# pdrebello/flash-attention-minitorch

Hardware: AMD Instinct MI355X
Metric: attn fw+bw TFLOP/s at (B=8,H=8,N=4096,d=64); % MFMA roofline (higher is better)
Workload: dtype bf16

## Files before the change

### flash_attention_minitorch_amd/csrc/fa_api.hip

```cpp
#include <hip/hip_runtime.h>
#include <math.h>
#include <algorithm>
#include <chrono>
#include <mutex>
#include <string>
#include <vector>
#include <stdio.h>
#include <stdlib.h>
#include <string.h>
#include <unistd.h>
#include <atomic>

#include "../../include/flash_attn_mi355x.h"
#include "fa_kernels.h"

namespace {

thread_local char g_err[512] = "";

int set_err(int code, const char* what, hipError_t e = hipSuccess) {
  if (e != hipSuccess)
    snprintf(g_err, sizeof(g_err), "%s: %s", what, hipGetErrorString(e));
  else
    snprintf(g_err, sizeof(g_err), "%s", what);
// ... 193 lines not shown
    m.check = false;
    s.add(Kern(base + 2), batch, 256, nqb, 0).twin_blocks = m.twin_blocks;
  }
}

template <typename T, int D>
Selection select_fwd(const Call& c) {
  constexpr bool BF = sizeof(T) == 2;
  const int batch = c.batch, N = c.N, causal = c.causal;
  const Tun& tun = c.tun;
  const bool plain = !c.lay.kmask && !c.lay.drop_thr;
  Selection s;
  if (!BF && D == 64) {
    const long wgs = (long)batch * ((N + 127) / 128), cus = device_cus();
    if (plain && !c.lay.out_bf16 && N >= 128 && (tun.v[1] == 4 ||
         (tun.v[1] == 0 && wgs <= (causal ? FWD_SPLITK_MAX_WGS_PER_CU_CAUSAL : FWD_SPLITK_MAX_WGS_PER_CU) * cus))) {
      const int nqb = (N + 31) / 32;
      s.add(FWD_SPLITK, batch * nqb, 256, nqb);
      return s;
    }
  }
  if (BF && (D == 64 || D == 128)) {
    const int nqb = (N + 255) / 256;
    const bool cslot = causal && N % 256 == 0 && (tun.v[1] == 3 || (tun.v[1] == 0 && batch * nqb >= 256));
    if (c.variant == FA_VARIANT_FA2 && tun.v[1] != 2 && (!causal || tun.v[1] == 3 || cslot) && plain && N >= 64) {
      if (cslot) {
        const bool ranked = causal_ranked(tun, batch * nqb, D == 64 ? 2 : 1);
        s.add(FWD_SLOT_CAUSAL, ranked ? batch * nqb : batch * ((nqb + 1) / 2), 512, nqb, ranked ? 2 : 1).rank_chunk =
            rank_chunk(D == 64 ? 2 : 1, nqb);
        s.folds = true;
        return s;
      }
      if (!causal && N % (8192 / D) == 0) {
        s.add(FWD_SLOT_WHOLE, batch * nqb, 512, nqb, causal);
        s.folds = s.produces_guard = true;
        return s;
      }
      if (D == 64) {
        s.add(FWD_SLOT_MASKED, batch * nqb, 512, nqb, causal);
        if (causal) select_phased(s, c, BF, FWD_DROP, 0, 0, 0, false);
        return s;
      }
    }
  }
  select_phased(s, c, BF, FWD_DROP, -1, D == 64 ? 1 : 0, tun.v[7] == 2 || (tun.v[7] == 0 && BF && D == 32), false);
  return s;
}

template <typename T, int D>
void select_dkdv_phased(Selection& s, const Call& c, bool mode3 = false, int care_main = 0, int rank_causal = 1) {
  constexpr bool BF = sizeof(T) == 2;
  constexpr int NW = BF ? 8 : 4;
  const int batch = c.batch, N = c.N, causal = c.causal;
  const int nkb = (N + NW * 32 - 1) / (NW * 32), nkb4 = (N + 127) / 128;
  const bool rank = causal && rank_causal;
  if (c.lay.drop_thr) {
    if (BF) s.add(DKDV_CARE_DROP, batch * nkb4, 256, nkb4).rank_chunk = rank ? rank_chunk(2, nkb4) : 0;
    else s.add(DKDV_DROP_F32, batch * nkb, NW * 64, nkb).rank_chunk = rank ? rank_chunk(2, nkb) : 0;
    return;
  }
  if (BF && (c.lay.kmask || N < 64)) {
    s.add(DKDV_CARE, batch * nkb4, 256, nkb4).rank_chunk = rank ? rank_chunk(2, nkb4) : 0;
    return;
  }
  if (mode3 && causal && care_main) {
    s.add(DKDV_CARE_MAIN, batch * ((nkb + 1) / 2), NW * 64, nkb);
    return;
// ... 149 lines not shown
#define FA_FWD_SLOT(...) FA_GO((fa::fwd_slot_kernel<__VA_ARGS__>), FA_QKV, c.out, c.l, N, s.nb, batch, lay, s.arg, c.tau)
#define FA_DQ(FEAT, NWQ, ...)                                                                                                    \
  FA_GO((fa::bwd_dq_kernel<T, D, 32, FEAT, NWQ, ##__VA_ARGS__>), FA_QKV, (const T*)c.dout, c.nlc(), c.delta(), c.dq, N, s.nb, batch, lay, \
        causal, c.tau, s.arg, pa)
#define FA_DQ_SLOT(...)                                                                                                            \
  FA_GO((fa::bwd_dq_slot_kernel<T, D, ##__VA_ARGS__>), FA_QKV, (const T*)c.dout, c.nlc(), c.delta(), c.dq, N, s.nb, batch, lay, s.arg, \
        c.tau, pa)
#define FA_DKDV_SLOT(...)                                                                                                         \
  FA_GO((fa::bwd_dkdv_slot_kernel<T, 64, ##__VA_ARGS__>), FA_QKV, (const T*)c.dout, c.nl2(), c.delta(), c.dk, c.dv, N, s.nb, batch, lay, \
        c.tau)
#define FA_DKDV(...)                                                                                                               \
  FA_GO((fa::bwd_dkdv_kernel<T, D, 32, __VA_ARGS__>), FA_QKV, (const T*)c.dout, c.nlc(), c.delta(), c.dk, c.dv, N, s.nb, batch, lay, \
        causal, c.tau, s.arg)
#define FA_ONEPASS(C, R)                                                                                                         \
  FA_GO((fa::bwd_onepass_f32_kernel<D, C, R>), FA_QKV, (const T*)c.dout, c.nlc(), c.delta(), c.dq, c.dk, c.dv, N, s.nb, batch, lay, \
        c.tau, s.arg)
  for (int i = 0; i < sel.n; ++i) {
    const Step& s = sel.steps[i];
    fa::Layout lay = c.lay;
    lay.rank_chunk = s.rank_chunk;
    lay.tiles = s.tiles;
    lay.twin_blocks = s.twin_blocks;
    lay.guard_want = s.guard_want;
    const fa::DqPrep pa = s.prep ? fa::DqPrep{c.out, c.l, c.m, c.nlc(), c.delta(), c.nl2(), c.variant, 1.0f / c.tau} : fa::DqPrep{};
    switch (s.kern) {
      case FWD_SPLITK:
        if constexpr (!BF && D == 64)
          FA_GO((fa::fwd_splitk_f32_kernel<D>), FA_QKV, c.out, c.l, c.m, N, s.nb, batch, lay, causal, c.variant, c.tau);
        break;
      case FWD_SLOT_CAUSAL:
        if constexpr (BF && D >= 64) FA_FWD_SLOT(T, D, false, 64, (D == 64 ? 4 : 2), true);
        break;
      case FWD_SLOT_WHOLE:
        if constexpr (BF && D == 64) FA_FWD_SLOT(T, 64, false, 64, 4);
        else if constexpr (BF && D == 128) FA_FWD_SLOT(T, D, false);
        break;
      case FWD_SLOT_MASKED:
        if constexpr (BF && D == 64) FA_FWD_SLOT(T, D, true);
        break;
      case FWD_DROP: FA_FWD(2, BF); break;
      case FWD_MASK: FA_FWD(1, BF); break;
      case FWD_CARE: FA_FWD(0, BF); break;
      case FWD_MAIN: FA_FWD(0, false); break;
      case BWD_PREP:
        FA_GO((fa::bwd_prep_kernel<T, D>), c.out, (const T*)c.dout, c.l, c.m, c.nlc(), c.delta(), c.nl2(), rows, N, lay, c.variant,
              1.0f / c.tau);
        break;
      case DQ_DROP: FA_DQ(2, 4, BF); break;
      case DQ_MASK: FA_DQ(1, 4, BF); break;
      case DQ_CARE: FA_DQ(0, 4, BF); break;
      case DQ_MAIN: FA_DQ(0, 4, false); break;
      case DQ_WAVE8:
        if constexpr (BF && D == 128) FA_DQ(0, 8);
        break;
      case DQ_SLOT_CAUSAL:
        if constexpr (BF && D == 64) FA_DQ_SLOT(false, true);
        break;
      case DQ_SLOT_TILED:
        if constexpr (BF && D == 64) FA_DQ_SLOT(false, false, true);
        break;
      case DQ_SLOT_WHOLE:
        if constexpr (BF && D == 64) FA_DQ_SLOT(false);
        break;
      case DQ_SLOT_MASKED:
        if constexpr (BF && D == 64) FA_DQ_SLOT();
        break;
      case DKDV_SLOT_TILED:
// ... 851 lines not shown
```

### flash_attention_minitorch_amd/csrc/fa_common.h

```cpp
#pragma once
#include <type_traits>

#include "fa_atoms.h"

namespace fa {

constexpr float LOG2E = 1.4426950408889634f;
constexpr int AUX_FA1 = 1;
constexpr int AUX_FA2 = 2;

template <int V> using ic = std::integral_constant<int, V>;

FA_DEV int lane_fresh() {
  int l;
  asm volatile("v_mbcnt_lo_u32_b32 %0, -1, 0\n\tv_mbcnt_hi_u32_b32 %0, -1, %0" : "=v"(l));
  return l;
}

template <typename T> FA_DEV typename Atom<T>::frag load_frag_buf(rsrc_t rs, int byte_off);
template <> FA_DEV bf16x8 load_frag_buf<bf16_t>(rsrc_t rs, int byte_off) {
  return __builtin_bit_cast(bf16x8, __builtin_amdgcn_raw_buffer_load_b128(rs, byte_off, 0, 0));
}
template <> FA_DEV f32x8 load_frag_buf<float>(rsrc_t rs, int byte_off) {
  f32x4 a = __builtin_bit_cast(f32x4, __builtin_amdgcn_raw_buffer_load_b128(rs, byte_off, 0, 0));
  f32x4 b = __builtin_bit_cast(f32x4, __builtin_amdgcn_raw_buffer_load_b128(rs, byte_off + 16, 0, 0));
  return __builtin_shufflevector(a, b, 0, 1, 2, 3, 4, 5, 6, 7);
}

constexpr int GUARD_SLOTS = 256;
FA_DEV bool guard_beyond(const Layout& L) {
  const int lane = threadIdx.x & 63;
  const f32x4 a = *reinterpret_cast<const f32x4*>(L.guard + 4 * lane);
  const f32x4 b = *reinterpret_cast<const f32x4*>(L.guard + GUARD_SLOTS + 4 * lane);
  float qm = fmaxf(fmaxf(a[0], a[1]), fmaxf(a[2], a[3])), km = fmaxf(fmaxf(b[0], b[1]), fmaxf(b[2], b[3]));
#pragma unroll
  for (int off = 32; off > 0; off >>= 1) {
    qm = fmaxf(qm, __shfl_xor(qm, off));
    km = fmaxf(km, __shfl_xor(km, off));
  }
  const bool beyond = !(L.guard_coef * __builtin_sqrtf(qm * km) <= 1.0f);
  return __builtin_amdgcn_readfirstlane((int)beyond) != 0;
}
FA_DEV bool guard_skip(const Layout& L) {
  if (L.guard == nullptr || L.guard_want >= 2) return false;
  return guard_beyond(L) != (L.guard_want != 0);
}
FA_DEV bool scale_exact(const Layout& L) {
  if (L.scale_sel != 2 || L.guard == nullptr) return L.scale_sel != 0;
  return guard_beyond(L);
}

FA_DEV bool guard_produce(const Layout& L, float qs, float ks, lds_char* scratch) {
  qs = xhalf_sum(qs);
  ks = xhalf_sum(ks);
#pragma unroll
  for (int off = 16; off > 0; off >>= 1) {
    qs = fmaxf(qs, __shfl_xor(qs, off));
    ks = fmaxf(ks, __shfl_xor(ks, off));
  }
  const int w = threadIdx.x >> 6;
  if ((threadIdx.x & 63) == 0) {
    unsigned* g = reinterpret_cast<unsigned*>(const_cast<float*>(L.guard)) + (blockIdx.x & (GUARD_SLOTS - 1));
    atomicMax(g, __float_as_uint(qs));
    atomicMax(g + GUARD_SLOTS, __float_as_uint(ks));
    *FA_LDS(float, scratch + 4 * w) = qs;
    *FA_LDS(float, scratch + 32 + 4 * w) = ks;
  }
  __syncthreads();
  float qm = 0.f, km = 0.f;
#pragma unroll
  for (int i = 0; i < 8; ++i) {
    qm = fmaxf(qm, *FA_LDS(float, scratch + 4 * i));
    km = fmaxf(km, *FA_LDS(float, scratch + 32 + 4 * i));
  }
  __syncthreads();
  return !(L.guard_coef * __builtin_sqrtf(qm * km) <= 1.0f);
}
template <typename F> FA_DEV float frag_sumsq(const F& f) {
  float s = 0.f;
#pragma unroll
  for (int j = 0; j < 8; ++j) s = __builtin_fmaf((float)f[j], (float)f[j], s);
  return s;
}

FA_DEV void store_out4(float* o, size_t elem_off, const f32x4& val, int out_bf16) {
  if (out_bf16) {
    *reinterpret_cast<bf16x4*>(reinterpret_cast<bf16_t*>(o) + elem_off) = __builtin_convertvector(val, bf16x4);
  } else {
    *reinterpret_cast<f32x4*>(o + elem_off) = val;
  }
}

FA_DEV f32x16 zero16() {
  f32x16 z;
#pragma unroll
  for (int i = 0; i < 16; ++i) z[i] = 0.f;
  return z;
}

}
```

### flash_attention_minitorch_amd/csrc/fa_fwd.h

```cpp
#pragma once
#include "fa_common.h"

namespace fa {

constexpr float MAX_DEFER_SUM = 64.0f;

template <typename T, int D, int BN, int WPE, int FEAT = 0, bool CARE = false>
__global__ void __launch_bounds__(256) __attribute__((amdgpu_waves_per_eu(WPE)))
fwd_kernel(const T* __restrict__ q, const T* __restrict__ k, const T* __restrict__ v, float* __restrict__ o,
           float* __restrict__ aux_l, float* __restrict__ aux_m, int N, int nqb, int BH, Layout lay, int causal,
           int aux_mode, float tau, int only_qb = -1) {
  if (guard_skip(lay)) return;
  using A = Atom<T>;
  typedef typename A::frag frag;
  constexpr bool HM = FEAT >= 1, HD = FEAT >= 2;
  constexpr int KC = D / 16, KT = BN / 32, DT = D / 32;
  constexpr int TB = A::template tile_bytes<D>(BN);
  __shared__ __attribute__((aligned(16))) char smem_raw[4 * TB];
  __shared__ __attribute__((aligned(16))) float smask[HM ? 2 * BN : 4];
  lds_char* smem = (lds_char*)smem_raw;

  const int tid = threadIdx.x, lane = tid & 63, r = lane & 31, h = lane >> 5;
  const int w = __builtin_amdgcn_readfirstlane(tid >> 6);
  const bool ranked = only_qb < 0 && causal && lay.rank_chunk > 0;
// ... 266 lines not shown
#pragma unroll
        for (int dt = 0; dt < DT; ++dt)
#pragma unroll
          for (int i = 0; i < 16; ++i) acc_o[dt][i] *= alpha;
        m_ref += delta;
      }
    }
    const float nm = -m_ref;
    float rs = 0.f;
#pragma unroll
    for (int i = 0; i < 16; ++i) {
      s[i] = __builtin_amdgcn_exp2f(__builtin_fmaf(s[i], c, nm));
      rs += s[i];
    }
    l_run = l_run * alpha + rs;
    const frag pf0 = A::pack(s, 0), pf1 = A::pack(s, 1);
    const frag pl0 = A::pack_lo(s, 0, pf0), pl1 = A::pack_lo(s, 1, pf1);
#pragma unroll
    for (int s2 = 0; s2 < 2; ++s2)
#pragma unroll
      for (int dt = 0; dt < DT; ++dt) {
        typedef __attribute__((ext_vector_type(8))) unsigned short u16x8;
        u16x8 raw;
#pragma unroll
        for (int j = 0; j < 8; ++j)
          raw[j] = __builtin_amdgcn_raw_buffer_load_b16(vrs, ((k0 + 16 * s2 + 8 * (j >> 2) + 4 * h + (j & 3)) * ldk + 32 * dt + r) * 2, 0, 0);
        const frag vt = __builtin_bit_cast(frag, raw);
        A::mma(acc_o[dt], vt, s2 ? pf1 : pf0);
        A::mma(acc_o[dt], vt, s2 ? pl1 : pl0);
      }
  }
}

template <typename T, int D, bool MASKS = true, int STK = 8192 / D, int MINW = 2, bool CDIAG = false>
__global__ void __launch_bounds__(512, MINW)
fwd_slot_kernel(const T* __restrict__ q, const T* __restrict__ k, const T* __restrict__ v, float* __restrict__ o,
                float* __restrict__ aux_l, int N, int nqb, int BH, Layout lay, int causal, float tau) {
  if (guard_skip(lay)) return;
  static_assert((D == 64 || D == 128) && sizeof(T) == 2, "slot schedule is laid out for bf16, d = 64 / 128");
  using A = Atom<T>;
  typedef typename A::frag frag;
  constexpr int KC = D / 16, DT = D / 32, NS = 2 * KC, EPS = 16 / NS;
  constexpr int ST = STK;
  constexpr int NSUBT = ST / 32;
  constexpr int R = NSUBT == 2 ? 4 : 3;
  constexpr int TB = A::template tile_bytes<D>(ST);
  constexpr int VOFF = R * TB;
  using RG = StageRing<D, ST>;
  static_assert(RG::dma_matches_image(), "LDS-DMA source swizzle vs Atom::off");
  static_assert((TB == 16384 || TB == 8192) && 2 * DT == KC && (NSUBT == 2 || NSUBT == 4), "stage geometry");
  static_assert(!CDIAG || (!MASKS && NSUBT == 2 && R * ST == 256), "causal build: the ring holds one 256-key diagonal block");
  constexpr bool PRE = !MASKS;
  __shared__ __attribute__((aligned(16))) char smem_raw[2 * R * TB];
  lds_char* smem = (lds_char*)smem_raw;

  const int tid = threadIdx.x, lane = tid & 63, r0_ = lane & 31, h0_ = lane >> 5;
  const int w = __builtin_amdgcn_readfirstlane(tid >> 6);
  const bool ranked = CDIAG && causal == 2;
  const int nblk = (CDIAG && !ranked) ? (nqb + 1) / 2 : nqb;
  int bh, pblk;
  if (ranked) map_block_ranked(blockIdx.x, BH, nblk, max(lay.rank_chunk, 1), bh, pblk);
  else map_block(blockIdx.x, BH, nblk, bh, pblk);
  const size_t base = head_base(lay, bh);
  const int ld = lay.ld;
  const uint32_t mat_bytes = ((uint32_t)(N - 1) * ld + D) * (uint32_t)sizeof(T);
  const rsrc_t qrs = make_rsrc(q + base, mat_bytes);
  const size_t kvb = kv_base<D>(lay, bh, N);
  const int ldk = lay.ldk;
  const uint32_t kv_bytes = ((uint32_t)(N - 1) * ldk + D) * (uint32_t)sizeof(T);
  const raw_rsrc_t kraw = make_raw_rsrc(k + kvb, kv_bytes), vraw = make_raw_rsrc(v + kvb, kv_bytes);
  const float c = tau * LOG2E;
  const int npass = (CDIAG && !ranked && pblk != nqb - 1 - pblk) ? 2 : 1;
  for (int pass = 0; pass < npass; ++pass) {
  const int qb = CDIAG ? (pass == 0 ? nqb - 1 - pblk : pblk) : (causal ? nqb - 1 - pblk : pblk);
  if (CDIAG && pass) __syncthreads();
  int r = r0_, h = h0_;
  if constexpr (CDIAG) {
    const int l2 = lane_fresh();
    r = l2 & 31;
    h = l2 >> 5;
  }
  const int q0 = qb * 256 + w * 32;
  int qrow = q0 + r;

  frag qf[KC];
  const bool produce = PRE && !CDIAG && lay.guard_want == 2 && lay.guard != nullptr;
  frag kg[KC];
  if (produce) {
    const rsrc_t krs = make_rsrc(k + kvb, kv_bytes);
#pragma unroll
    for (int kc = 0; kc < KC; ++kc) kg[kc] = load_frag_buf<T>(krs, (qrow * ldk + 16 * kc + 8 * h) * (int)sizeof(T));
  }
#pragma unroll
  for (int kc = 0; kc < KC; ++kc) qf[kc] = load_frag_buf<T>(qrs, (qrow * ld + 16 * kc + 8 * h) * (int)sizeof(T));
  const bool exactq = CDIAG && A::SPLITS && q0 < 64;
  const float cm = (PRE && !exactq) ? 1.0f : c;
  f32x16 acc_o[DT];
#pragma unroll
  for (int dt = 0; dt < DT; ++dt) acc_o[dt] = zero16();
  float m_ref = 0.f, nmc = 0.f, l_run = 0.f;

  const LaneAddr ra = A::template row_addr<D>(lane);
  const LaneAddr ta = A::template tr_addr<D>(lane);
  const int kmax = CDIAG ? qb * 256 : (causal ? min(N, qb * 256 + 256) : N);
  const int nstage = (kmax + ST - 1) / ST;
  const uint32_t smem_addr = (uint32_t)(uintptr_t)smem;
  FA_DMA_VOFF(dma_voff, RG::PPG, lane, w, ldk, (int)sizeof(T));
  auto stage_dma = [&](int row0, int slot_base) {
#pragma unroll
    for (int g2 = 0; g2 < RG::NPW; ++g2) {
      const int piece = w + 8 * g2, g = piece / RG::PPG;
      const int soff = (row0 + 8 * g) * ldk * (int)sizeof(T);
      dma16(kraw, smem_addr + slot_base + 1024 * piece, dma_voff, soff);
      dma16(vraw, smem_addr + slot_base + VOFF + 1024 * piece, dma_voff, soff);
    }
  };
  if constexpr (MASKS) {
#pragma unroll 4
    for (int off = tid * 16; off < 2 * R * TB; off += 512 * 16) *FA_LDS(u32x4, smem + off) = u32x4{0u, 0u, 0u, 0u};
    __syncthreads();
  }
  const int nst_w = CDIAG ? nstage + (w >> 1) : nstage;
  const int nst_all = CDIAG ? nstage + 3 : nstage;
  {
  stage_dma(0, 0);
  if (NSUBT == 2 && (CDIAG || nstage > 1)) stage_dma(ST, ring_slot<R, TB>(1));
  if (produce) {
    float qs = 0.f, ks = 0.f;
#pragma unroll
    for (int kc = 0; kc < KC; ++kc) {
      qs += frag_sumsq(qf[kc]);
      ks += frag_sumsq(kg[kc]);
    }
    if (guard_produce(lay, qs, ks, smem + 2 * R * TB - 64)) {
      dma_wait_all();
      return;
    }
  }
  if (PRE && !exactq) {
#pragma unroll
    for (int kc = 0; kc < KC; ++kc) qf[kc] = A::scale(qf[kc], c);
  }
  dma_wait_all();
  __syncthreads();

  if (lay.young_prio && w >= 4) __builtin_amdgcn_s_setprio(1);
  f32x16 sA, sB;
  u32x4 pA0, pA1, pB0, pB1;
  frag rk[4], tf[4];
  auto SB = [&]() { __builtin_amdgcn_sched_barrier(0); };
  auto cvt2 = [&](float a, float b) -> uint32_t {
    f32x2 pr = {a, b};
    return __builtin_bit_cast(uint32_t, __builtin_convertvector(pr, bf16x2));
  };
  auto mask_scores = [&](f32x16& x, int kcur) {
    const int klim = causal ? (min(qrow, N - 1) - kcur) : (N - 1 - kcur);
#pragma unroll
    for (int i = 0; i < 16; ++i)
      if (acc_row(i, h) > klim) x[i] = -INFINITY;
  };
  auto tile_max = [&](const f32x16& x) {
    float mx = x[0];
#pragma unroll
    for (int i = 1; i < 16; ++i) mx = fmaxf(mx, x[i]);
    return xhalf_max(mx);
  };
  auto period = [&](auto hn_c, auto hc_c, auto hp_c, auto mask_c, auto subn_c, auto subp_c, auto sub2_c, auto subc_c,
                    int rn0, int rn1, int tp0, int tp1, int r20, int r21, int rc0, int rc1, int kcur, f32x16& ns,
                    f32x16& cs, u32x4& pp0, u32x4& pp1, u32x4& pc0, u32x4& pc1) {
    constexpr bool HN = decltype(hn_c)::value != 0, HC = decltype(hc_c)::value != 0, HP = decltype(hp_c)::value != 0;
    constexpr bool MASK = decltype(mask_c)::value != 0;
    constexpr int SUBN = decltype(subn_c)::value, SUBP = decltype(subp_c)::value, SUB2 = decltype(sub2_c)::value;
    constexpr int SUBC = decltype(subc_c)::value;
    float rs = 0.f, cm = c;
    if constexpr (MASK) {
      asm volatile("" : "+v"(cm));
      if constexpr (HC) mask_scores(cs, kcur);
    }
    auto fe = [&](int i) {
      const float pv = PRE ? __builtin_amdgcn_exp2f(cs[i]) : __builtin_amdgcn_exp2f(__builtin_fmaf(cs[i], cm, nmc));
      cs[i] = pv;
      rs += pv;
    };
    auto valu = [&](int g) {
      if constexpr (HC) {
#pragma unroll
        for (int e = 0; e < EPS; ++e) fe(g * EPS + e);
#pragma unroll
        for (int p = 0; p < 8; ++p) {
          const int done_at = (2 * p + 1) / EPS;
          if (done_at == g - 1 || (g == NS - 1 && done_at == g)) {
            const uint32_t pk = cvt2(cs[2 * p], cs[2 * p + 1]);
            if (p < 4) pc0[p] = pk;
            else pc1[p - 4] = pk;
          }
        }
      }
    };
#pragma unroll
    for (int kq = 0; kq < KC; ++kq) {
      if constexpr (HN) {
        if (kq == 0) A::mma_c(ns, rk[0], qf[0], zero16());
        else A::mma(ns, rk[kq & 3], qf[kq]);
        SB();
        if (kq + 2 < KC) rk[(kq + 2) & 3] = RG::row(smem, rn0, rn1, SUBN, kq + 2);
      }
      valu(kq);
      if constexpr (HP) {
        if (kq >= KC - 2) tf[kq - (KC - 2)] = RG::tr(smem, tp0, tp1, SUBP, 0, kq - (KC - 2), VOFF);
      }
      SB();
    }
#pragma unroll
    for (int t = 0; t < KC; ++t) {
      if constexpr (HP) {
        A::mma(acc_o[t % DT], tf[t & 3], __builtin_bit_cast(frag, (t < DT) ? pp0 : pp1));
        SB();
        if (t + 2 < KC) tf[(t + 2) & 3] = RG::tr(smem, tp0, tp1, SUBP, (t + 2) / DT, (t + 2) % DT, VOFF);
      }
      valu(KC + t);
      if constexpr (HN) {
        if (t >= KC - 2) rk[t - (KC - 2)] = RG::row(smem, r20, r21, SUB2, t - (KC - 2));
      }
      SB();
    }
    if constexpr (HC && PRE) l_run += rs;
    if constexpr (HC && !PRE) {
      float alpha = 1.0f;
      if (__any(!(rs < MAX_DEFER_SUM))) {
#pragma unroll
        for (int kc = 0; kc < KC; ++kc) {
          const frag kk = RG::row(smem, rc0, rc1, SUBC, kc);
          if (kc == 0) A::mma_c(cs, kk, qf[0], zero16());
          else A::mma(cs, kk, qf[kc]);
        }
        if constexpr (MASK) mask_scores(cs, kcur);
        const float delta = fmaxf(tile_max(cs) - m_ref, 0.f);
        alpha = __builtin_amdgcn_exp2f(-delta * c);
#pragma unroll
        for (int dt = 0; dt < DT; ++dt)
#pragma unroll
          for (int i = 0; i < 16; ++i) acc_o[dt][i] *= alpha;
        m_ref += delta;
        nmc = -m_ref * c;
        rs = 0.f;
#pragma unroll
        for (int i = 0; i < 16; ++i) {
          cs[i] = __builtin_amdgcn_exp2f(__builtin_fmaf(cs[i], c, nmc));
          rs += cs[i];
        }
#pragma unroll
        for (int j = 0; j < 4; ++j) {
          pc0[j] = cvt2(cs[2 * j], cs[2 * j + 1]);
          pc1[j] = cvt2(cs[8 + 2 * j], cs[9 + 2 * j]);
        }
      }
      l_run = l_run * alpha + rs;
    }
  };
  auto T1 = ic<1>{};
  auto T0 = ic<0>{};
  int cr0 = ra.b[0], cr1 = ra.b[1];
  int ct0 = ta.b[0], ct1 = ta.b[1];
  int pt0 = ct0, pt1 = ct1;
  rk[0] = RG::row(smem, cr0, cr1, 0, 0);
  rk[1] = RG::row(smem, cr0, cr1, 0, 1);
  pB0 = pB1 = pA0 = pA1 = u32x4{0u, 0u, 0u, 0u};
  SB();
  period(T1, T0, T0, T0, ic<0>{}, ic<0>{}, ic<1>{}, ic<0>{}, cr0, cr1, ct0, ct1, cr0, cr1, cr0, cr1, 0, sA, sB, pB0, pB1, pA0, pA1);
  if constexpr (!PRE) {
    const bool m0 = MASKS && ((31 >= N) || (causal && 31 > q0));
    if (m0) mask_scores(sA, 0);
    m_ref = tile_max(sA);
    nmc = -m_ref * c;
  }
  for (int st = 0; st < nst_w; ++st) {
    const int nb = ring_slot<R, TB>(st + 1);
    const int nr0 = ra.b[0] + nb, nr1 = ra.b[1] + nb;
    const int kb = st * ST;
    auto need = [&](int sub) { return MASKS && ((kb + 32 * sub + 31 >= N) || (causal && kb + 32 * sub + 31 > q0)); };
    if constexpr (NSUBT == 4) {
      if (st + 1 < nstage) stage_dma((st + 1) * ST, nb);
      if constexpr (MASKS) {
        if (need(0)) period(T1, T1, T1, T1, ic<1>{}, ic<3>{}, ic<2>{}, ic<0>{}, cr0, cr1, pt0, pt1, cr0, cr1, cr0, cr1, kb, sB, sA, pB0, pB1, pA0, pA1);
        else period(T1, T1, T1, T0, ic<1>{}, ic<3>{}, ic<2>{}, ic<0>{}, cr0, cr1, pt0, pt1, cr0, cr1, cr0, cr1, kb, sB, sA, pB0, pB1, pA0, pA1);
      } else {
        period(T1, T1, T1, T0, ic<1>{}, ic<3>{}, ic<2>{}, ic<0>{}, cr0, cr1, pt0, pt1, cr0, cr1, cr0, cr1, kb, sB, sA, pB0, pB1, pA0, pA1);
      }
      if constexpr (MASKS) {
        if (need(1)) period(T1, T1, T1, T1, ic<2>{}, ic<0>{}, ic<3>{}, ic<1>{}, cr0, cr1, ct0, ct1, cr0, cr1, cr0, cr1, kb + 32, sA, sB, pA0, pA1, pB0, pB1);
        else period(T1, T1, T1, T0, ic<2>{}, ic<0>{}, ic<3>{}, ic<1>{}, cr0, cr1, ct0, ct1, cr0, cr1, cr0, cr1, kb + 32, sA, sB, pA0, pA1, pB0, pB1);
      } else {
        period(T1, T1, T1, T0, ic<2>{}, ic<0>{}, ic<3>{}, ic<1>{}, cr0, cr1, ct0, ct1, cr0, cr1, cr0, cr1, kb + 32, sA, sB, pA0, pA1, pB0, pB1);
      }
      dma_wait_all();
      __syncthreads();
      if constexpr (MASKS) {
        if (need(2)) period(T1, T1, T1, T1, ic<3>{}, ic<1>{}, ic<0>{}, ic<2>{}, cr0, cr1, ct0, ct1, nr0, nr1, cr0, cr1, kb + 64, sB, sA, pB0, pB1, pA0, pA1);
        else period(T1, T1, T1, T0, ic<3>{}, ic<1>{}, ic<0>{}, ic<2>{}, cr0, cr1, ct0, ct1, nr0, nr1, cr0, cr1, kb + 64, sB, sA, pB0, pB1, pA0, pA1);
      } else {
        period(T1, T1, T1, T0, ic<3>{}, ic<1>{}, ic<0>{}, ic<2>{}, cr0, cr1, ct0, ct1, nr0, nr1, cr0, cr1, kb + 64, sB, sA, pB0, pB1, pA0, pA1);
      }
      if constexpr (MASKS) {
        if (need(3)) period(T1, T1, T1, T1, ic<0>{}, ic<2>{}, ic<1>{}, ic<3>{}, nr0, nr1, ct0, ct1, nr0, nr1, cr0, cr1, kb + 96, sA, sB, pA0, pA1, pB0, pB1);
        else period(T1, T1, T1, T0, ic<0>{}, ic<2>{}, ic<1>{}, ic<3>{}, nr0, nr1, ct0, ct1, nr0, nr1, cr0, cr1, kb + 96, sA, sB, pA0, pA1, pB0, pB1);
      } else {
        period(T1, T1, T1, T0, ic<0>{}, ic<2>{}, ic<1>{}, ic<3>{}, nr0, nr1, ct0, ct1, nr0, nr1, cr0, cr1, kb + 96, sA, sB, pA0, pA1, pB0, pB1);
      }
    } else {
      if (st > 0) {
        dma_wait_all();
        __syncthreads();
      }
      if (CDIAG ? st + 2 < nstage + 4 : st + 2 < nstage) stage_dma((st + 2) * ST, ring_slot<R, TB>(st + 2));
      if constexpr (MASKS) {
        if (need(0)) period(T1, T1, T1, T1, ic<1>{}, ic<1>{}, ic<0>{}, ic<0>{}, cr0, cr1, pt0, pt1, nr0, nr1, cr0, cr1, kb, sB, sA, pB0, pB1, pA0, pA1);
        else period(T1, T1, T1, T0, ic<1>{}, ic<1>{}, ic<0>{}, ic<0>{}, cr0, cr1, pt0, pt1, nr0, nr1, cr0, cr1, kb, sB, sA, pB0, pB1, pA0, pA1);
      } else {
        period(T1, T1, T1, T0, ic<1>{}, ic<1>{}, ic<0>{}, ic<0>{}, cr0, cr1, pt0, pt1, nr0, nr1, cr0, cr1, kb, sB, sA, pB0, pB1, pA0, pA1);
      }
      if constexpr (MASKS) {
        if (need(1)) period(T1, T1, T1, T1, ic<0>{}, ic<0>{}, ic<1>{}, ic<1>{}, nr0, nr1, ct0, ct1, nr0, nr1, cr0, cr1, kb + 32, sA, sB, pA0, pA1, pB0, pB1);
        else period(T1, T1, T1, T0, ic<0>{}, ic<0>{}, ic<1>{}, ic<1>{}, nr0, nr1, ct0, ct1, nr0, nr1, cr0, cr1, kb + 32, sA, sB, pA0, pA1, pB0, pB1);
      } else {
        period(T1, T1, T1, T0, ic<0>{}, ic<0>{}, ic<1>{}, ic<1>{}, nr0, nr1, ct0, ct1, nr0, nr1, cr0, cr1, kb + 32, sA, sB, pA0, pA1, pB0, pB1);
      }
    }
    pt0 = ct0; pt1 = ct1;
    cr0 = nr0; cr1 = nr1;
    ct0 = ta.b[0] + nb; ct1 = ta.b[1] + nb;
  }
  period(T0, T0, T1, T0, ic<0>{}, ic<NSUBT - 1>{}, ic<0>{}, ic<0>{}, cr0, cr1, pt0, pt1, cr0, cr1, cr0, cr1, 0, sB, sA, pB0, pB1, pA0, pA1);
  if constexpr (CDIAG) {
    if (nst_w == 0) {
#pragma unroll
      for (int dt = 0; dt < DT; ++dt) acc_o[dt] = zero16();
    }
  }
  if constexpr (CDIAG) {
    for (int st = nst_w; st < nst_all; ++st) {
      if (st > 0) {
        dma_wait_all();
        __syncthreads();
      }
      if (st + 2 < nstage + 4) stage_dma((st + 2) * ST, ring_slot<R, TB>(st + 2));
    }
  }
  }

  if constexpr (CDIAG) {
    {
      const int l2 = lane_fresh();
      r = l2 & 31;
      h = l2 >> 5;
      qrow = q0 + r;
    }
    const bool careful = exactq;
    auto diag_tile = [&](int j, bool first) {
      f32x16 s;
#pragma unroll
      for (int kc = 0; kc < KC; ++kc) {
        const frag kk = A::template row_frag<D>(smem, ra, 32 * j, kc);
        if (kc == 0) A::mma_c(s, kk, qf[0], zero16());
        else A::mma(s, kk, qf[kc]);
      }
      if (j == w) {
#pragma unroll
        for (int i = 0; i < 16; ++i)
          if (acc_row(i, h) > r) s[i] = -INFINITY;
      }
      float mx = s[0];
#pragma unroll
      for (int i = 1; i < 16; ++i) mx = fmaxf(mx, s[i]);
      mx = xhalf_max(mx) * cm;
      float alpha = 1.0f;
      if (first) {
        m_ref = mx;
      } else {
        const float delta = fmaxf(mx - m_ref, 0.f);
        if (__any(delta > 0.f)) {
          alpha = __builtin_amdgcn_exp2f(-delta);
#pragma unroll
          for (int dt = 0; dt < DT; ++dt)
#pragma unroll
            for (int i = 0; i < 16; ++i) acc_o[dt][i] *= alpha;
          m_ref += delta;
        }
      }
      nmc = -m_ref;
      float rs = 0.f;
#pragma unroll
      for (int i = 0; i < 16; ++i) {
        s[i] = __builtin_amdgcn_exp2f(__builtin_fmaf(s[i], cm, nmc));
        rs += s[i];
      }
      l_run = l_run * alpha + rs;
      const frag pf0 = A::pack(s, 0), pf1 = A::pack(s, 1);
      if (!careful) {
#pragma unroll
        for (int s2 = 0; s2 < 2; ++s2)
#pragma unroll
          for (int dt = 0; dt < DT; ++dt)
            A::mma(acc_o[dt], A::template tr_frag<D>(smem + VOFF, ta, 32 * j + 16 * s2, dt), s2 ? pf1 : pf0);
      } else {
        const frag pl0 = A::pack_lo(s, 0, pf0), pl1 = A::pack_lo(s, 1, pf1);
#pragma unroll
        for (int s2 = 0; s2 < 2; ++s2)
#pragma unroll
          for (int dt = 0; dt < DT; ++dt) {
            const frag vt = A::template tr_frag<D>(smem + VOFF, ta, 32 * j + 16 * s2, dt);
            A::mma(acc_o[dt], vt, s2 ? pf1 : pf0);
            A::mma(acc_o[dt], vt, s2 ? pl1 : pl0);
          }
      }
    };
    for (int j = 2 * (w >> 1); j <= w; ++j) diag_tile(j, nst_w == 0 && j == 0);
  }

  float l_tot = xhalf_sum(l_run);
  if constexpr (PRE) {
    if (__any(!(l_tot >= 0x1p-96f && l_tot <= 0x1p96f))) {
      if constexpr (CDIAG) {
        const int l2 = lane_fresh();
        r = l2 & 31;
        h = l2 >> 5;
        qrow = q0 + r;
      }
      fwd_redo_rows<D>(qrs, make_rsrc(k + kvb, kv_bytes), make_rsrc(v + kvb, kv_bytes), qrow, q0, ld, ldk, N, CDIAG, c, r, h, acc_o,
                       m_ref, l_run);
      l_tot = xhalf_sum(l_run);
    }
  }
  const float inv = 1.0f / l_tot;
  int qr = qrow, hh = h;
  if constexpr (CDIAG) {
    const int l2 = lane_fresh();
    qr = q0 + (l2 & 31);
    hh = l2 >> 5;
  } else {
    asm volatile("" : "+v"(qr), "+v"(hh));
  }
  if (qr < N) {
    const size_t orow = base + (size_t)qr * ld;
#pragma unroll
    for (int dt = 0; dt < DT; ++dt)
#pragma unroll
      for (int g = 0; g < 4; ++g) {
        f32x4 val = {acc_o[dt][4 * g] * inv, acc_o[dt][4 * g + 1] * inv, acc_o[dt][4 * g + 2] * inv,
                     acc_o[dt][4 * g + 3] * inv};
        store_out4(o, orow + 32 * dt + 8 * g + 4 * hh, val, lay.out_bf16);
      }
    if (hh == 0)
      aux_l[(size_t)bh * N + qr] = PRE ? (m_ref + __builtin_amdgcn_logf(l_tot)) * 0.6931471805599453f : m_ref * tau + __logf(l_tot);
  }
  }
}


}
```

Measured before the change: 878.4.

## Process two 32-row query groups per wave in non-causal d=64 forward slot kernel

The mask-free non-causal d=64 forward slot kernel now has each wave own two 32-row query groups, so the block shrinks from 8 to 4 waves (256 threads). Each K/V fragment read from LDS is reused for two row groups, which cuts LDS traffic per MFMA. The K and V DMA for the next stage is split around the two halves of the period so it overlaps compute. The cost is doubled accumulator and score registers per wave, which can lower occupancy or cause spills. The guard reduction is generalised to a variable wave count.

After: 876.4. Within noise of the previous version (-0.2%).

```diff
diff --git a/flash_attention_minitorch_amd/csrc/fa_api.hip b/flash_attention_minitorch_amd/csrc/fa_api.hip
--- a/flash_attention_minitorch_amd/csrc/fa_api.hip
+++ b/flash_attention_minitorch_amd/csrc/fa_api.hip
@@ -249,7 +249,7 @@
         return s;
       }
       if (!causal && N % (8192 / D) == 0) {
-        s.add(FWD_SLOT_WHOLE, batch * nqb, 512, nqb, causal);
+        s.add(FWD_SLOT_WHOLE, batch * nqb, D == 64 ? 256 : 512, nqb, causal);
         s.folds = s.produces_guard = true;
         return s;
       }
@@ -465,7 +465,7 @@
         if constexpr (BF && D >= 64) FA_FWD_SLOT(T, D, false, 64, (D == 64 ? 4 : 2), true);
         break;
       case FWD_SLOT_WHOLE:
-        if constexpr (BF && D == 64) FA_FWD_SLOT(T, 64, false, 64, 4);
+        if constexpr (BF && D == 64) FA_FWD_SLOT(T, 64, false, 64, 2, false, 2);
         else if constexpr (BF && D == 128) FA_FWD_SLOT(T, D, false);
         break;
       case FWD_SLOT_MASKED:
diff --git a/flash_attention_minitorch_amd/csrc/fa_common.h b/flash_attention_minitorch_amd/csrc/fa_common.h
--- a/flash_attention_minitorch_amd/csrc/fa_common.h
+++ b/flash_attention_minitorch_amd/csrc/fa_common.h
@@ -50,9 +50,8 @@
   return guard_beyond(L);
 }
 
-FA_DEV bool guard_produce(const Layout& L, float qs, float ks, lds_char* scratch) {
-  qs = xhalf_sum(qs);
-  ks = xhalf_sum(ks);
+template <int NW>
+FA_DEV bool guard_produce_rows(const Layout& L, float qs, float ks, lds_char* scratch) {
 #pragma unroll
   for (int off = 16; off > 0; off >>= 1) {
     qs = fmaxf(qs, __shfl_xor(qs, off));
@@ -69,12 +68,15 @@
   __syncthreads();
   float qm = 0.f, km = 0.f;
 #pragma unroll
-  for (int i = 0; i < 8; ++i) {
+  for (int i = 0; i < NW; ++i) {
     qm = fmaxf(qm, *FA_LDS(float, scratch + 4 * i));
     km = fmaxf(km, *FA_LDS(float, scratch + 32 + 4 * i));
   }
   __syncthreads();
   return !(L.guard_coef * __builtin_sqrtf(qm * km) <= 1.0f);
+}
+FA_DEV bool guard_produce(const Layout& L, float qs, float ks, lds_char* scratch) {
+  return guard_produce_rows<8>(L, xhalf_sum(qs), xhalf_sum(ks), scratch);
 }
 template <typename F> FA_DEV float frag_sumsq(const F& f) {
   float s = 0.f;
diff --git a/flash_attention_minitorch_amd/csrc/fa_fwd.h b/flash_attention_minitorch_amd/csrc/fa_fwd.h
--- a/flash_attention_minitorch_amd/csrc/fa_fwd.h
+++ b/flash_attention_minitorch_amd/csrc/fa_fwd.h
@@ -322,8 +322,8 @@
   }
 }
 
-template <typename T, int D, bool MASKS = true, int STK = 8192 / D, int MINW = 2, bool CDIAG = false>
-__global__ void __launch_bounds__(512, MINW)
+template <typename T, int D, bool MASKS = true, int STK = 8192 / D, int MINW = 2, bool CDIAG = false, int NG = 1>
+__global__ void __launch_bounds__(512 / NG, MINW)
 fwd_slot_kernel(const T* __restrict__ q, const T* __restrict__ k, const T* __restrict__ v, float* __restrict__ o,
                 float* __restrict__ aux_l, int N, int nqb, int BH, Layout lay, int causal, float tau) {
   if (guard_skip(lay)) return;
@@ -336,7 +336,9 @@
   constexpr int R = NSUBT == 2 ? 4 : 3;
   constexpr int TB = A::template tile_bytes<D>(ST);
   constexpr int VOFF = R * TB;
-  using RG = StageRing<D, ST>;
+  constexpr int NW = 8 / NG;
+  using RG = StageRing<D, ST, NW>;
+  static_assert(NG == 1 || (NG == 2 && D == 64 && !MASKS && !CDIAG), "two row groups per wave: the mask-free non-causal d = 64 build");
   static_assert(RG::dma_matches_image(), "LDS-DMA source swizzle vs Atom::off");
   static_assert((TB == 16384 || TB == 8192) && 2 * DT == KC && (NSUBT == 2 || NSUBT == 4), "stage geometry");
   static_assert(!CDIAG || (!MASKS && NSUBT == 2 && R * ST == 256), "causal build: the ring holds one 256-key diagonal block");
@@ -370,25 +372,37 @@
     r = l2 & 31;
     h = l2 >> 5;
   }
-  const int q0 = qb * 256 + w * 32;
+  const int q0 = qb * 256 + w * (32 * NG);
   int qrow = q0 + r;
 
-  frag qf[KC];
+  frag qf[NG][KC];
   const bool produce = PRE && !CDIAG && lay.guard_want == 2 && lay.guard != nullptr;
-  frag kg[KC];
+  frag kg[NG][KC];
   if (produce) {
     const rsrc_t krs = make_rsrc(k + kvb, kv_bytes);
 #pragma unroll
-    for (int kc = 0; kc < KC; ++kc) kg[kc] = load_frag_buf<T>(krs, (qrow * ldk + 16 * kc + 8 * h) * (int)sizeof(T));
-  }
-#pragma unroll
-  for (int kc = 0; kc < KC; ++kc) qf[kc] = load_frag_buf<T>(qrs, (qrow * ld + 16 * kc + 8 * h) * (int)sizeof(T));
+    for (int kc = 0; kc < KC; ++kc) kg[0][kc] = load_frag_buf<T>(krs, (qrow * ldk + 16 * kc + 8 * h) * (int)sizeof(T));
+    if constexpr (NG == 2) {
+#pragma unroll
+      for (int kc = 0; kc < KC; ++kc) kg[1][kc] = load_frag_buf<T>(krs, ((qrow + 32) * ldk + 16 * kc + 8 * h) * (int)sizeof(T));
+    }
+  }
+#pragma unroll
+  for (int kc = 0; kc < KC; ++kc) qf[0][kc] = load_frag_buf<T>(qrs, (qrow * ld + 16 * kc + 8 * h) * (int)sizeof(T));
+  if constexpr (NG == 2) {
+#pragma unroll
+    for (int kc = 0; kc < KC; ++kc) qf[1][kc] = load_frag_buf<T>(qrs, ((qrow + 32) * ld + 16 * kc + 8 * h) * (int)sizeof(T));
+  }
   const bool exactq = CDIAG && A::SPLITS && q0 < 64;
   const float cm = (PRE && !exactq) ? 1.0f : c;
-  f32x16 acc_o[DT];
-#pragma unroll
-  for (int dt = 0; dt < DT; ++dt) acc_o[dt] = zero16();
-  float m_ref = 0.f, nmc = 0.f, l_run = 0.f;
+  f32x16 acc_o[NG][DT];
+  float m_ref[NG], l_run[NG], nmc = 0.f;
+#pragma unroll
+  for (int g = 0; g < NG; ++g) {
+#pragma unroll
+    for (int dt = 0; dt < DT; ++dt) acc_o[g][dt] = zero16();
+    m_ref[g] = l_run[g] = 0.f;
+  }
 
   const LaneAddr ra = A::template row_addr<D>(lane);
   const LaneAddr ta = A::template tr_addr<D>(lane);
@@ -399,10 +413,17 @@
   auto stage_dma = [&](int row0, int slot_base) {
 #pragma unroll
     for (int g2 = 0; g2 < RG::NPW; ++g2) {
-      const int piece = w + 8 * g2, g = piece / RG::PPG;
+      const int piece = w + NW * g2, g = piece / RG::PPG;
       const int soff = (row0 + 8 * g) * ldk * (int)sizeof(T);
       dma16(kraw, smem_addr + slot_base + 1024 * piece, dma_voff, soff);
       dma16(vraw, smem_addr + slot_base + VOFF + 1024 * piece, dma_voff, soff);
+    }
+  };
+  auto stage_dma_half = [&](int row0, int slot_base, const raw_rsrc_t& rs, int toff) {
+#pragma unroll
+    for (int g2 = 0; g2 < RG::NPW; ++g2) {
+      const int piece = w + NW * g2, g = piece / RG::PPG;
+      dma16(rs, smem_addr + slot_base + toff + 1024 * piece, dma_voff, (row0 + 8 * g) * ldk * (int)sizeof(T));
     }
   };
   if constexpr (MASKS) {
@@ -416,27 +437,40 @@
   stage_dma(0, 0);
   if (NSUBT == 2 && (CDIAG || nstage > 1)) stage_dma(ST, ring_slot<R, TB>(1));
   if (produce) {
-    float qs = 0.f, ks = 0.f;
-#pragma unroll
-    for (int kc = 0; kc < KC; ++kc) {
-      qs += frag_sumsq(qf[kc]);
-      ks += frag_sumsq(kg[kc]);
-    }
-    if (guard_produce(lay, qs, ks, smem + 2 * R * TB - 64)) {
+    float qs[NG], ks[NG];
+#pragma unroll
+    for (int g = 0; g < NG; ++g) {
+      qs[g] = ks[g] = 0.f;
+#pragma unroll
+      for (int kc = 0; kc < KC; ++kc) {
+        qs[g] += frag_sumsq(qf[g][kc]);
+        ks[g] += frag_sumsq(kg[g][kc]);
+      }
+    }
+    bool beyond;
+    if constexpr (NG == 1) {
+      beyond = guard_produce(lay, qs[0], ks[0], smem + 2 * R * TB - 64);
+    } else {
+      beyond = guard_produce_rows<NW>(lay, fmaxf(xhalf_sum(qs[0]), xhalf_sum(qs[1])), fmaxf(xhalf_sum(ks[0]), xhalf_sum(ks[1])),
+                                      smem + 2 * R * TB - 64);
+    }
+    if (beyond) {
       dma_wait_all();
       return;
     }
   }
   if (PRE && !exactq) {
 #pragma unroll
-    for (int kc = 0; kc < KC; ++kc) qf[kc] = A::scale(qf[kc], c);
+    for (int g = 0; g < NG; ++g)
+#pragma unroll
+      for (int kc = 0; kc < KC; ++kc) qf[g][kc] = A::scale(qf[g][kc], c);
   }
   dma_wait_all();
   __syncthreads();
 
-  if (lay.young_prio && w >= 4) __builtin_amdgcn_s_setprio(1);
-  f32x16 sA, sB;
-  u32x4 pA0, pA1, pB0, pB1;
+  if (lay.young_prio && w >= NW / 2) __builtin_amdgcn_s_setprio(1);
+  f32x16 sA[NG], sB[NG];
+  u32x4 pA0[NG], pA1[NG], pB0[NG], pB1[NG];
   frag rk[4], tf[4];
   auto SB = [&]() { __builtin_amdgcn_sched_barrier(0); };
   auto cvt2 = [&](float a, float b) -> uint32_t {
@@ -456,96 +490,107 @@
     return xhalf_max(mx);
   };
   auto period = [&](auto hn_c, auto hc_c, auto hp_c, auto mask_c, auto subn_c, auto subp_c, auto sub2_c, auto subc_c,
-                    int rn0, int rn1, int tp0, int tp1, int r20, int r21, int rc0, int rc1, int kcur, f32x16& ns,
-                    f32x16& cs, u32x4& pp0, u32x4& pp1, u32x4& pc0, u32x4& pc1) {
+                    int rn0, int rn1, int tp0, int tp1, int r20, int r21, int rc0, int rc1, int kcur, f32x16 (&ns)[NG],
+                    f32x16 (&cs)[NG], u32x4 (&pp0)[NG], u32x4 (&pp1)[NG], u32x4 (&pc0)[NG], u32x4 (&pc1)[NG]) {
     constexpr bool HN = decltype(hn_c)::value != 0, HC = decltype(hc_c)::value != 0, HP = decltype(hp_c)::value != 0;
     constexpr bool MASK = decltype(mask_c)::value != 0;
     constexpr int SUBN = decltype(subn_c)::value, SUBP = decltype(subp_c)::value, SUB2 = decltype(sub2_c)::value;
     constexpr int SUBC = decltype(subc_c)::value;
-    float rs = 0.f, cm = c;
+    float rs[NG], cm = c;
+#pragma unroll
+    for (int g = 0; g < NG; ++g) rs[g] = 0.f;
     if constexpr (MASK) {
       asm volatile("" : "+v"(cm));
-      if constexpr (HC) mask_scores(cs, kcur);
-    }
-    auto fe = [&](int i) {
-      const float pv = PRE ? __builtin_amdgcn_exp2f(cs[i]) : __builtin_amdgcn_exp2f(__builtin_fmaf(cs[i], cm, nmc));
-      cs[i] = pv;
-      rs += pv;
+      if constexpr (HC) mask_scores(cs[0], kcur);
+    }
+    auto fe = [&](int g, int i) {
+      const float pv = PRE ? __builtin_amdgcn_exp2f(cs[g][i]) : __builtin_amdgcn_exp2f(__builtin_fmaf(cs[g][i], cm, nmc));
+      cs[g][i] = pv;
+      rs[g] += pv;
     };
-    auto valu = [&](int g) {
+    auto valu = [&](int g, int sl) {
       if constexpr (HC) {
 #pragma unroll
-        for (int e = 0; e < EPS; ++e) fe(g * EPS + e);
+        for (int e = 0; e < EPS; ++e) fe(g, sl * EPS + e);
 #pragma unroll
         for (int p = 0; p < 8; ++p) {
           const int done_at = (2 * p + 1) / EPS;
-          if (done_at == g - 1 || (g == NS - 1 && done_at == g)) {
-            const uint32_t pk = cvt2(cs[2 * p], cs[2 * p + 1]);
-            if (p < 4) pc0[p] = pk;
-            else pc1[p - 4] = pk;
+          if (done_at == sl - 1 || (sl == NS - 1 && done_at == sl)) {
+            const uint32_t pk = cvt2(cs[g][2 * p], cs[g][2 * p + 1]);
+            if (p < 4) pc0[g][p] = pk;
+            else pc1[g][p - 4] = pk;
           }
         }
       }
     };
 #pragma unroll
     for (int kq = 0; kq < KC; ++kq) {
-      if constexpr (HN) {
-        if (kq == 0) A::mma_c(ns, rk[0], qf[0], zero16());
-        else A::mma(ns, rk[kq & 3], qf[kq]);
+#pragma unroll
+      for (int g = 0; g < NG; ++g) {
+        if constexpr (HN) {
+          if (kq == 0) A::mma_c(ns[g], rk[0], qf[g][0], zero16());
+          else A::mma(ns[g], rk[kq & 3], qf[g][kq]);
+          SB();
+          if (g == NG - 1 && kq + 2 < KC) rk[(kq + 2) & 3] = RG::row(smem, rn0, rn1, SUBN, kq + 2);
+        }
+        valu(g, kq);
+        if constexpr (HP) {
+          if (g == NG - 1 && kq >= KC - 2) tf[kq - (KC - 2)] = RG::tr(smem, tp0, tp1, SUBP, 0, kq - (KC - 2), VOFF);
+        }
         SB();
-        if (kq + 2 < KC) rk[(kq + 2) & 3] = RG::row(smem, rn0, rn1, SUBN, kq + 2);
-      }
-      valu(kq);
-      if constexpr (HP) {
-        if (kq >= KC - 2) tf[kq - (KC - 2)] = RG::tr(smem, tp0, tp1, SUBP, 0, kq - (KC - 2), VOFF);
-      }
-      SB();
+      }
     }
 #pragma unroll
     for (int t = 0; t < KC; ++t) {
-      if constexpr (HP) {
-        A::mma(acc_o[t % DT], tf[t & 3], __builtin_bit_cast(frag, (t < DT) ? pp0 : pp1));
+#pragma unroll
+      for (int g = 0; g < NG; ++g) {
+        if constexpr (HP) {
+          A::mma(acc_o[g][t % DT], tf[t & 3], __builtin_bit_cast(frag, (t < DT) ? pp0[g] : pp1[g]));
+          SB();
+          if (g == NG - 1 && t + 2 < KC) tf[(t + 2) & 3] = RG::tr(smem, tp0, tp1, SUBP, (t + 2) / DT, (t + 2) % DT, VOFF);
+        }
+        valu(g, KC + t);
+        if constexpr (HN) {
+          if (g == NG - 1 && t >= KC - 2) rk[t - (KC - 2)] = RG::row(smem, r20, r21, SUB2, t - (KC - 2));
+        }
         SB();
-        if (t + 2 < KC) tf[(t + 2) & 3] = RG::tr(smem, tp0, tp1, SUBP, (t + 2) / DT, (t + 2) % DT, VOFF);
-      }
-      valu(KC + t);
-      if constexpr (HN) {
-        if (t >= KC - 2) rk[t - (KC - 2)] = RG::row(smem, r20, r21, SUB2, t - (KC - 2));
-      }
-      SB();
-    }
-    if constexpr (HC && PRE) l_run += rs;
+      }
+    }
+    if constexpr (HC && PRE) {
+#pragma unroll
+      for (int g = 0; g < NG; ++g) l_run[g] += rs[g];
+    }
     if constexpr (HC && !PRE) {
       float alpha = 1.0f;
-      if (__any(!(rs < MAX_DEFER_SUM))) {
+      if (__any(!(rs[0] < MAX_DEFER_SUM))) {
 #pragma unroll
         for (int kc = 0; kc < KC; ++kc) {
           const frag kk = RG::row(smem, rc0, rc1, SUBC, kc);
-          if (kc == 0) A::mma_c(cs, kk, qf[0], zero16());
-          else A::mma(cs, kk, qf[kc]);
-        }
-        if constexpr (MASK) mask_scores(cs, kcur);
-        const float delta = fmaxf(tile_max(cs) - m_ref, 0.f);
+          if (kc == 0) A::mma_c(cs[0], kk, qf[0][0], zero16());
+          else A::mma(cs[0], kk, qf[0][kc]);
+        }
+        if constexpr (MASK) mask_scores(cs[0], kcur);
+        const float delta = fmaxf(tile_max(cs[0]) - m_ref[0], 0.f);
         alpha = __builtin_amdgcn_exp2f(-delta * c);
 #pragma unroll
         for (int dt = 0; dt < DT; ++dt)
 #pragma unroll
-          for (int i = 0; i < 16; ++i) acc_o[dt][i] *= alpha;
-        m_ref += delta;
-        nmc = -m_ref * c;
-        rs = 0.f;
+          for (int i = 0; i < 16; ++i) acc_o[0][dt][i] *= alpha;
+        m_ref[0] += delta;
+        nmc = -m_ref[0] * c;
+        rs[0] = 0.f;
 #pragma unroll
         for (int i = 0; i < 16; ++i) {
-          cs[i] = __builtin_amdgcn_exp2f(__builtin_fmaf(cs[i], c, nmc));
-          rs += cs[i];
+          cs[0][i] = __builtin_amdgcn_exp2f(__builtin_fmaf(cs[0][i], c, nmc));
+          rs[0] += cs[0][i];
         }
 #pragma unroll
         for (int j = 0; j < 4; ++j) {
-          pc0[j] = cvt2(cs[2 * j], cs[2 * j + 1]);
-          pc1[j] = cvt2(cs[8 + 2 * j], cs[9 + 2 * j]);
-        }
-      }
-      l_run = l_run * alpha + rs;
+          pc0[0][j] = cvt2(cs[0][2 * j], cs[0][2 * j + 1]);
+          pc1[0][j] = cvt2(cs[0][8 + 2 * j], cs[0][9 + 2 * j]);
+        }
+      }
+      l_run[0] = l_run[0] * alpha + rs[0];
     }
   };
   auto T1 = ic<1>{};
@@ -555,14 +600,15 @@
   int pt0 = ct0, pt1 = ct1;
   rk[0] = RG::row(smem, cr0, cr1, 0, 0);
   rk[1] = RG::row(smem, cr0, cr1, 0, 1);
-  pB0 = pB1 = pA0 = pA1 = u32x4{0u, 0u, 0u, 0u};
+#pragma unroll
+  for (int g = 0; g < NG; ++g) pB0[g] = pB1[g] = pA0[g] = pA1[g] = u32x4{0u, 0u, 0u, 0u};
   SB();
   period(T1, T0, T0, T0, ic<0>{}, ic<0>{}, ic<1>{}, ic<0>{}, cr0, cr1, ct0, ct1, cr0, cr1, cr0, cr1, 0, sA, sB, pB0, pB1, pA0, pA1);
   if constexpr (!PRE) {
     const bool m0 = MASKS && ((31 >= N) || (causal && 31 > q0));
-    if (m0) mask_scores(sA, 0);
-    m_ref = tile_max(sA);
-    nmc = -m_ref * c;
+    if (m0) mask_scores(sA[0], 0);
+    m_ref[0] = tile_max(sA[0]);
+    nmc = -m_ref[0] * c;
   }
   for (int st = 0; st < nst_w; ++st) {
     const int nb = ring_slot<R, TB>(st + 1);
@@ -602,13 +648,20 @@
         dma_wait_all();
         __syncthreads();
       }
-      if (CDIAG ? st + 2 < nstage + 4 : st + 2 < nstage) stage_dma((st + 2) * ST, ring_slot<R, TB>(st + 2));
+      if constexpr (NG == 2) {
+        if (st + 2 < nstage) stage_dma_half((st + 2) * ST, ring_slot<R, TB>(st + 2), kraw, 0);
+      } else {
+        if (CDIAG ? st + 2 < nstage + 4 : st + 2 < nstage) stage_dma((st + 2) * ST, ring_slot<R, TB>(st + 2));
+      }
       if constexpr (MASKS) {
         if (need(0)) period(T1, T1, T1, T1, ic<1>{}, ic<1>{}, ic<0>{}, ic<0>{}, cr0, cr1, pt0, pt1, nr0, nr1, cr0, cr1, kb, sB, sA, pB0, pB1, pA0, pA1);
         else period(T1, T1, T1, T0, ic<1>{}, ic<1>{}, ic<0>{}, ic<0>{}, cr0, cr1, pt0, pt1, nr0, nr1, cr0, cr1, kb, sB, sA, pB0, pB1, pA0, pA1);
       } else {
         period(T1, T1, T1, T0, ic<1>{}, ic<1>{}, ic<0>{}, ic<0>{}, cr0, cr1, pt0, pt1, nr0, nr1, cr0, cr1, kb, sB, sA, pB0, pB1, pA0, pA1);
       }
+      if constexpr (NG == 2) {
+        if (st + 2 < nstage) stage_dma_half((st + 2) * ST, ring_slot<R, TB>(st + 2), vraw, VOFF);
+      }
       if constexpr (MASKS) {
         if (need(1)) period(T1, T1, T1, T1, ic<0>{}, ic<0>{}, ic<1>{}, ic<1>{}, nr0, nr1, ct0, ct1, nr0, nr1, cr0, cr1, kb + 32, sA, sB, pA0, pA1, pB0, pB1);
         else period(T1, T1, T1, T0, ic<0>{}, ic<0>{}, ic<1>{}, ic<1>{}, nr0, nr1, ct0, ct1, nr0, nr1, cr0, cr1, kb + 32, sA, sB, pA0, pA1, pB0, pB1);
@@ -624,7 +677,7 @@
   if constexpr (CDIAG) {
     if (nst_w == 0) {
 #pragma unroll
-      for (int dt = 0; dt < DT; ++dt) acc_o[dt] = zero16();
+      for (int dt = 0; dt < DT; ++dt) acc_o[0][dt] = zero16();
     }
   }
   if constexpr (CDIAG) {
@@ -651,8 +704,8 @@
 #pragma unroll
       for (int kc = 0; kc < KC; ++kc) {
         const frag kk = A::template row_frag<D>(smem, ra, 32 * j, kc);
-        if (kc == 0) A::mma_c(s, kk, qf[0], zero16());
-        else A::mma(s, kk, qf[kc]);
+        if (kc == 0) A::mma_c(s, kk, qf[0][0], zero16());
+        else A::mma(s, kk, qf[0][kc]);
       }
       if (j == w) {
 #pragma unroll
@@ -665,33 +718,33 @@
       mx = xhalf_max(mx) * cm;
       float alpha = 1.0f;
       if (first) {
-        m_ref = mx;
-      } else {
-        const float delta = fmaxf(mx - m_ref, 0.f);
+        m_ref[0] = mx;
+      } else {
+        const float delta = fmaxf(mx - m_ref[0], 0.f);
         if (__any(delta > 0.f)) {
           alpha = __builtin_amdgcn_exp2f(-delta);
 #pragma unroll
           for (int dt = 0; dt < DT; ++dt)
 #pragma unroll
-            for (int i = 0; i < 16; ++i) acc_o[dt][i] *= alpha;
-          m_ref += delta;
-        }
-      }
-      nmc = -m_ref;
+            for (int i = 0; i < 16; ++i) acc_o[0][dt][i] *= alpha;
+          m_ref[0] += delta;
+        }
+      }
+      nmc = -m_ref[0];
       float rs = 0.f;
 #pragma unroll
       for (int i = 0; i < 16; ++i) {
         s[i] = __builtin_amdgcn_exp2f(__builtin_fmaf(s[i], cm, nmc));
         rs += s[i];
       }
-      l_run = l_run * alpha + rs;
+      l_run[0] = l_run[0] * alpha + rs;
       const frag pf0 = A::pack(s, 0), pf1 = A::pack(s, 1);
       if (!careful) {
 #pragma unroll
         for (int s2 = 0; s2 < 2; ++s2)
 #pragma unroll
           for (int dt = 0; dt < DT; ++dt)
-            A::mma(acc_o[dt], A::template tr_frag<D>(smem + VOFF, ta, 32 * j + 16 * s2, dt), s2 ? pf1 : pf0);
+            A::mma(acc_o[0][dt], A::template tr_frag<D>(smem + VOFF, ta, 32 * j + 16 * s2, dt), s2 ? pf1 : pf0);
       } else {
         const frag pl0 = A::pack_lo(s, 0, pf0), pl1 = A::pack_lo(s, 1, pf1);
 #pragma unroll
@@ -699,15 +752,18 @@
 #pragma unroll
           for (int dt = 0; dt < DT; ++dt) {
             const frag vt = A::template tr_frag<D>(smem + VOFF, ta, 32 * j + 16 * s2, dt);
-            A::mma(acc_o[dt], vt, s2 ? pf1 : pf0);
-            A::mma(acc_o[dt], vt, s2 ? pl1 : pl0);
+            A::mma(acc_o[0][dt], vt, s2 ? pf1 : pf0);
+            A::mma(acc_o[0][dt], vt, s2 ? pl1 : pl0);
           }
       }
     };
     for (int j = 2 * (w >> 1); j <= w; ++j) diag_tile(j, nst_w == 0 && j == 0);
   }
 
-  float l_tot = xhalf_sum(l_run);
+#pragma unroll
+  for (int g = 0; g < NG; ++g) {
+  const int GR = 32 * g;
+  float l_tot = xhalf_sum(l_run[g]);
   if constexpr (PRE) {
     if (__any(!(l_tot >= 0x1p-96f && l_tot <= 0x1p96f))) {
       if constexpr (CDIAG) {
@@ -716,13 +772,13 @@
         h = l2 >> 5;
         qrow = q0 + r;
       }
-      fwd_redo_rows<D>(qrs, make_rsrc(k + kvb, kv_bytes), make_rsrc(v + kvb, kv_bytes), qrow, q0, ld, ldk, N, CDIAG, c, r, h, acc_o,
-                       m_ref, l_run);
-      l_tot = xhalf_sum(l_run);
+      fwd_redo_rows<D>(qrs, make_rsrc(k + kvb, kv_bytes), make_rsrc(v + kvb, kv_bytes), qrow + GR, q0 + GR, ld, ldk, N, CDIAG, c, r, h, acc_o[g],
+                       m_ref[g], l_run[g]);
+      l_tot = xhalf_sum(l_run[g]);
     }
   }
   const float inv = 1.0f / l_tot;
-  int qr = qrow, hh = h;
+  int qr = qrow + GR, hh = h;
   if constexpr (CDIAG) {
     const int l2 = lane_fresh();
     qr = q0 + (l2 & 31);
@@ -735,13 +791,15 @@
 #pragma unroll
     for (int dt = 0; dt < DT; ++dt)
 #pragma unroll
-      for (int g = 0; g < 4; ++g) {
-        f32x4 val = {acc_o[dt][4 * g] * inv, acc_o[dt][4 * g + 1] * inv, acc_o[dt][4 * g + 2] * inv,
-                     acc_o[dt][4 * g + 3] * inv};
-        store_out4(o, orow + 32 * dt + 8 * g + 4 * hh, val, lay.out_bf16);
+      for (int g4 = 0; g4 < 4; ++g4) {
+        f32x4 val = {acc_o[g][dt][4 * g4] * inv, acc_o[g][dt][4 * g4 + 1] * inv, acc_o[g][dt][4 * g4 + 2] * inv,
+                     acc_o[g][dt][4 * g4 + 3] * inv};
+        store_out4(o, orow + 32 * dt + 8 * g4 + 4 * hh, val, lay.out_bf16);
       }
     if (hh == 0)
-      aux_l[(size_t)bh * N + qr] = PRE ? (m_ref + __builtin_amdgcn_logf(l_tot)) * 0.6931471805599453f : m_ref * tau + __logf(l_tot);
+      aux_l[(size_t)bh * N + qr] =
+          PRE ? (m_ref[g] + __builtin_amdgcn_logf(l_tot)) * 0.6931471805599453f : m_ref[g] * tau + __logf(l_tot);
+  }
   }
   }
 }
```
